# malak29/video-text-detection-system

Hardware: AMD Instinct MI355X
Metric: frames/sec (detect+recognize) @720p, 1/2/4/8 MI355X; box IoU vs CPU ref (higher is better)
Workload: dtype f16

## Files before the change

### include/vtd.h

```cpp
#ifndef VTD_H
#define VTD_H

#include <stddef.h>
#include <stdint.h>

#ifdef __cplusplus
extern "C" {
#endif

typedef struct vtd_detector vtd_detector;
typedef struct vtd_recognizer vtd_recognizer;
typedef struct vtd_postproc vtd_postproc;
typedef void* vtd_stream;

typedef struct vtd_detection {
    int32_t bbox[4];
    int32_t polygon[8];
    float confidence;
    float area;
    int32_t first_x, first_y;
} vtd_detection;

const char* vtd_version(void);
const char* vtd_strerror(int code);
int vtd_device_count(void);

int vtd_detector_create(const char* backbone, int max_batch, vtd_detector** out);
void vtd_detector_destroy(vtd_detector* d);
int vtd_detector_set_tensor(vtd_detector* d, const char* key, const float* host_data, int64_t numel);
int vtd_detector_set_option(vtd_detector* d, const char* name, int value);
int vtd_detector_finalize(vtd_detector* d, vtd_stream stream);
int vtd_detector_preprocess(vtd_detector* d, const uint8_t* frames_dev, int n, int height, int width, vtd_stream stream);
int vtd_detector_set_input_nchw(vtd_detector* d, const float* x_dev, int n, vtd_stream stream);
int vtd_detector_forward(vtd_detector* d, int n, float* prob_dev, float* thresh_dev, vtd_stream stream);
int vtd_detector_read_tap(vtd_detector* d, const char* name, int n, float* host_out, int64_t capacity, vtd_stream stream);
int64_t vtd_detector_macs_per_frame(const vtd_detector* d);
int vtd_detector_set_profiling(vtd_detector* d, int enable);
int vtd_detector_num_ops(const vtd_detector* d);
int vtd_detector_get_profile(vtd_detector* d, int op_index, char* name, int name_cap, double* total_ms, int64_t* calls,
                             double* total_macs, vtd_stream stream);

int vtd_detector_set_tuning(vtd_detector* d, const char* table_text);
int64_t vtd_detector_get_tuning(const vtd_detector* d, char* buf, int64_t capacity);
int vtd_detector_tuning_measured(const vtd_detector* d);

int vtd_postproc_create(int max_batch, int map_h, int map_w, int max_out, vtd_postproc** out);
void vtd_postproc_destroy(vtd_postproc* pp);
int vtd_postproc_run(vtd_postproc* pp, const float* prob_dev, int n, const int32_t* orig_w_host, const int32_t* orig_h_host,
                     float threshold, vtd_detection* out_dev, int32_t* counts_dev, vtd_stream stream);
int vtd_copy_to_pinned_host(const void* src_dev, void* dst_pinned_host, int64_t bytes, vtd_stream stream);

int64_t vtd_dbloss_workspace_bytes(void);
int vtd_dbloss_forward(const float* prob_dev, const float* thresh_dev, const float* prob_target_dev, const float* thresh_target_dev, int64_t numel,
                       float smooth, void* workspace_dev, float* out4_dev, double* sums5_dev, vtd_stream stream);
int vtd_dbloss_backward(const float* prob_dev, const float* thresh_dev, const float* prob_target_dev, const float* thresh_target_dev, int64_t numel,
                        float smooth, const double* sums5_dev, const float* grad_out4_dev, float* grad_prob_dev, float* grad_thresh_dev,
                        vtd_stream stream);
int vtd_binary_counts_accumulate(const float* pred_dev, const float* target_dev, int64_t numel, float threshold, int64_t* counts4_dev,
                                 vtd_stream stream);

#define VTD_ADAMW_SLICE 64
#define VTD_ADAMW_CHUNK 4096
typedef struct vtd_adamw_tensor {
    float* p;
    const float* g;
// ... 176 lines not shown
```

### video-text-detection-system_amd/csrc/detector_misc.hip

```cpp
#include "vtd_common.h"

namespace {

constexpr int PRE_TY = 16;
constexpr int PRE_OUT = 640;
constexpr int PRE_CHUNK = 4;
#ifndef VTD_PRE_NT
#define VTD_PRE_NT 640
#endif
constexpr int PRE_NT = VTD_PRE_NT;
constexpr int PRE_COLS = (PRE_OUT + PRE_NT - 1) / PRE_NT;

struct PreParams {
    const uint8_t* frames;
    half_t* out;
    const int* xb;
    const int* xk;
    const int* yb;
    const int* yk;
    int H, W, ksx, ksy;
    int max_rows;
    unsigned quads_magic;
};

// ... 188 lines not shown
        uint32_t acc[4][3];
#pragma unroll
        for (int q = 0; q < 4; ++q)
#pragma unroll
            for (int c = 0; c < 3; ++c) acc[q][c] = 1u << 21;
#pragma unroll
        for (int t = 0; t < KSY; ++t) {
            const uint32_t kv = (uint32_t)yt[2 + t];
            const int r = min(ymin + t, nrows - 1);
            const uint4 px = *(const uint4*)(rows + r * PRE_OUT + g * 4);
            const uint32_t pv[4] = {px.x, px.y, px.z, px.w};
#pragma unroll
            for (int q = 0; q < 4; ++q) {
                acc[q][0] = __umul24(pv[q] & 0xffu, kv) + acc[q][0];
                acc[q][1] = __umul24((pv[q] >> 8) & 0xffu, kv) + acc[q][1];
                acc[q][2] = __umul24(pv[q] >> 16, kv) + acc[q][2];
            }
        }
        half8 o01, o23;
#pragma unroll
        for (int q = 0; q < 4; ++q) {
            const half_t h0 = lut[clip8_22((int)acc[q][2])];
            const half_t h1 = lut[256 + clip8_22((int)acc[q][1])];
            const half_t h2 = lut[512 + clip8_22((int)acc[q][0])];
            if (q < 2) { o01[q * 4] = h0; o01[q * 4 + 1] = h1; o01[q * 4 + 2] = h2; o01[q * 4 + 3] = (half_t)0.f; }
            else { o23[(q - 2) * 4] = h0; o23[(q - 2) * 4 + 1] = h1; o23[(q - 2) * 4 + 2] = h2; o23[(q - 2) * 4 + 3] = (half_t)0.f; }
        }
        half_t* dst = p.out + (((int64_t)img * 646 + oy + 3) * 646 + g * 4 + 3) * 4;
        *(half4*)(dst) = half4{o01[0], o01[1], o01[2], o01[3]};
        *(half4*)(dst + 4) = half4{o01[4], o01[5], o01[6], o01[7]};
        *(half4*)(dst + 8) = half4{o23[0], o23[1], o23[2], o23[3]};
        *(half4*)(dst + 12) = half4{o23[4], o23[5], o23[6], o23[7]};
    }
}

__global__ void nchw_to_input_kernel(const float* __restrict__ x, half_t* __restrict__ out, int n) {
    const int64_t idx = (int64_t)blockIdx.x * blockDim.x + threadIdx.x;
    const int64_t total = (int64_t)n * 640 * 640;
    if (idx >= total) return;
    const int img = (int)(idx / (640 * 640));
    const int rem = (int)(idx - (int64_t)img * 640 * 640);
    const int y = rem / 640, xx = rem - y * 640;
    const float* base = x + (int64_t)img * 3 * 640 * 640 + rem;
    half4 o = {(half_t)base[0], (half_t)base[640 * 640], (half_t)base[2 * 640 * 640], (half_t)0.f};
    *(half4*)(out + (((int64_t)img * 646 + y + 3) * 646 + xx + 3) * 4) = o;
}

struct PoolParams {
    const half_t* in;
    half_t* out;
    int n, c, ho, wo;
    int in_hp, in_wp, in_y0, in_x0;
    int out_hp, out_wp, out_ring;
    int kh, kw, sh, sw;
};

__global__ void maxpool_kernel(const PoolParams p) {
    const int cg = p.c >> 3;
    const int64_t total = (int64_t)p.n * p.ho * p.wo * cg;
    for (int64_t idx = (int64_t)blockIdx.x * blockDim.x + threadIdx.x; idx < total; idx += (int64_t)gridDim.x * blockDim.x) {
        const int g = (int)(idx % cg);
        int64_t t = idx / cg;
        const int ox = (int)(t % p.wo);
        t /= p.wo;
        const int oy = (int)(t % p.ho);
        const int img = (int)(t / p.ho);
// ... 18 lines not shown
    PreParams p{frames, out, xb, xk, yb, yk, H, W, ksx, ksy, max_rows, 0u};
    if ((W & 3) == 0 && W <= 2048 && ksy == 5 && (ksx == 5 || ksx == 7)) {
        const int lds_fast = (max_rows * PRE_OUT + PRE_CHUNK * (W + ksx) + PRE_TY * (2 + ksy)) * 4 + 3 * 256 * 2;
        p.quads_magic = (unsigned)(((1ull << 32) + (W / 4) - 1) / (W / 4));
        if (lds_fast <= 160 * 1024) {
            static bool attr5 = false, attr7 = false;
            if (ksx == 5) {
                if (!attr5) {
                    VTD_HIP_CHECK(hipFuncSetAttribute((const void*)preprocess_fast_kernel<5, 5>, hipFuncAttributeMaxDynamicSharedMemorySize, 160 * 1024));
                    attr5 = true;
                }
                hipLaunchKernelGGL((preprocess_fast_kernel<5, 5>), dim3(PRE_OUT / PRE_TY, n), dim3(PRE_NT), lds_fast, stream, p);
            } else {
                if (!attr7) {
                    VTD_HIP_CHECK(hipFuncSetAttribute((const void*)preprocess_fast_kernel<7, 5>, hipFuncAttributeMaxDynamicSharedMemorySize, 160 * 1024));
                    attr7 = true;
                }
                hipLaunchKernelGGL((preprocess_fast_kernel<7, 5>), dim3(PRE_OUT / PRE_TY, n), dim3(PRE_NT), lds_fast, stream, p);
            }
            return -(int)hipGetLastError();
        }
    }
    const int lds = ((max_rows * PRE_OUT * 3 + 15) & ~15) + PRE_CHUNK * ((W * 3 + 15) & ~15);
    if (lds > 160 * 1024) return -1010;
    static bool attr_done = false;
    if (!attr_done) {
        VTD_HIP_CHECK(hipFuncSetAttribute((const void*)preprocess_kernel, hipFuncAttributeMaxDynamicSharedMemorySize, 160 * 1024));
        attr_done = true;
    }
    hipLaunchKernelGGL(preprocess_kernel, dim3(PRE_OUT / PRE_TY, n), dim3(256), lds, stream, p);
    return -(int)hipGetLastError();
}

int vtd_launch_nchw_to_input(const float* x, half_t* out, int n, hipStream_t stream) {
    const int64_t total = (int64_t)n * 640 * 640;
    hipLaunchKernelGGL(nchw_to_input_kernel, dim3((unsigned)((total + 255) / 256)), dim3(256), 0, stream, x, out, n);
    return -(int)hipGetLastError();
}

int vtd_launch_maxpool(const TensorDesc& in, const TensorDesc& out, int n, int kh, int kw, int sh, int sw, int pad_h, int pad_w,
                       hipStream_t stream) {
    if (in.c != out.c || (in.c & 7)) return -1020;
    if (in.ring < pad_h || in.ring < pad_w) return -1021;
    if ((out.h - 1) * sh - pad_h + kh > in.h + (in.hp - in.h - in.ring) || (out.w - 1) * sw - pad_w + kw > in.w + (in.wp - in.w - in.ring))
        return -1022;
    PoolParams p{in.ptr, out.ptr, n, in.c, out.h, out.w, in.hp, in.wp, in.ring - pad_h, in.ring - pad_w,
                 out.hp, out.wp, out.ring, kh, kw, sh, sw};
    const int64_t total = (int64_t)n * out.h * out.w * (in.c >> 3);
    const int blocks = (int)((total + 255) / 256 < 256 * 16 ? (total + 255) / 256 : 256 * 16);
    hipLaunchKernelGGL(maxpool_kernel, dim3(blocks), dim3(256), 0, stream, p);
    return -(int)hipGetLastError();
}
```

### video-text-detection-system_amd/csrc/recognizer.hip

```cpp
#include "../../include/vtd.h"
#include "vtd_common.h"

namespace {

struct CropParams {
    const uint8_t* frames;
    const int32_t* boxes;
    uint8_t* out;
    int H, W, ncrops;
};

__device__ __forceinline__ void linear_coef(int ssize, int dsize, int d, int& ofs, int& c0, int& c1) {
    const double scale = 1.0 / ((double)dsize / (double)ssize);
    float f = (float)(((double)d + 0.5) * scale - 0.5);
    int s = (int)floorf(f);
    f -= (float)s;
    if (s < 0) { f = 0.f; s = 0; }
    if (s >= ssize - 1) { f = 0.f; s = ssize - 1; }
    ofs = s;
    c0 = __float2int_rn((1.f - f) * 2048.f);
    c1 = __float2int_rn(f * 2048.f);
}

__global__ __launch_bounds__(256) void crop_resize_kernel(const CropParams p) {
    const int crop = blockIdx.x;
    const int32_t* b = p.boxes + crop * 5;
    const int x1 = b[1], y1 = b[2], sw = b[3] - b[1], sh = b[4] - b[2];
    uint8_t* dst = p.out + (int64_t)crop * 32 * 128 * 3;
    if (sw <= 0 || sh <= 0 || b[0] < 0 || x1 < 0 || y1 < 0 || b[3] > p.W || b[4] > p.H) {
        for (int i = threadIdx.x; i < 32 * 128 * 3; i += 256) dst[i] = 0;
        return;
    }
    const uint8_t* src = p.frames + ((int64_t)b[0] * p.H + y1) * p.W * 3 + (int64_t)x1 * 3;
    const int64_t stride = (int64_t)p.W * 3;
    const bool area = (sw == 256 && sh == 64);
    for (int i = threadIdx.x; i < 32 * 128; i += 256) {
        const int dy = i >> 7, dx = i & 127;
        if (area) {
            const uint8_t* r0 = src + (int64_t)(2 * dy) * stride + (2 * dx) * 3;
            const uint8_t* r1 = r0 + stride;
#pragma unroll
            for (int c = 0; c < 3; ++c) dst[i * 3 + c] = (uint8_t)((r0[c] + r0[3 + c] + r1[c] + r1[3 + c] + 2) >> 2);
            continue;
        }
        int sx0, a0, a1, sy0, b0, b1;
        linear_coef(sw, 128, dx, sx0, a0, a1);
        linear_coef(sh, 32, dy, sy0, b0, b1);
        const int sx1 = min(sx0 + 1, sw - 1), sy1 = min(sy0 + 1, sh - 1);
        const uint8_t* r0 = src + (int64_t)sy0 * stride;
        const uint8_t* r1 = src + (int64_t)sy1 * stride;
#pragma unroll
        for (int c = 0; c < 3; ++c) {
            const int h0 = r0[sx0 * 3 + c] * a0 + r0[sx1 * 3 + c] * a1;
            const int h1 = r1[sx0 * 3 + c] * a0 + r1[sx1 * 3 + c] * a1;
            int v = (((b0 * (h0 >> 4)) >> 16) + ((b1 * (h1 >> 4)) >> 16) + 2) >> 2;
            dst[i * 3 + c] = (uint8_t)(v < 0 ? 0 : (v > 255 ? 255 : v));
        }
    }
}

struct Conv1Params {
    const uint8_t* in_u8;
    const float* in_f32;
    const half_t* w;
    const float* bias;
    half_t* out;
    int n;
};

__global__ __launch_bounds__(256) void crnn_conv1_pool_kernel(const Conv1Params p) {
    __shared__ __attribute__((aligned(16))) half_t atile[256 * 32];
    __shared__ half_t tile[4][130][4];
    const int crop = blockIdx.y, py = blockIdx.x;
    for (int i = threadIdx.x; i < 4 * 130 * 3; i += 256) {
        const int c = i % 3, xx = (i / 3) % 130, r = i / (3 * 130);
        const int y = 2 * py - 1 + r, x = xx - 1;
        float v = 0.f;
        if (y >= 0 && y < 32 && x >= 0 && x < 128) {
            if (p.in_u8) v = (float)p.in_u8[(((int64_t)crop * 32 + y) * 128 + x) * 3 + c] / 255.0f;
            else v = p.in_f32[(((int64_t)crop * 3 + c) * 32 + y) * 128 + x];
        }
        tile[r][xx][c] = (half_t)v;
    }
    __syncthreads();
    {
        const int t = threadIdx.x, w = t >> 6, member = (t >> 4) & 3, win = t & 15;
        const int oy = member >> 1, ox = 2 * (w * 16 + win) + (member & 1);
        half_t vals[32];
#pragma unroll
// ... 244 lines not shown
```

### video-text-detection-system_amd/csrc/vtd_api.cpp

```cpp
#include <algorithm>
#include <cmath>
#include <cstdio>
#include <cstdlib>
#include <cstring>
#include <map>
#include <memory>
#include <string>
#include <vector>

#include "../../include/vtd.h"
#include "vtd_common.h"

int vtd_launch_conv(const ConvParams& p, int cfg, hipStream_t stream);
int vtd_conv_num_configs();
bool vtd_conv_config_valid(const ConvParams& p, int cfg);
int vtd_launch_preprocess(const uint8_t* frames, int n, int H, int W, half_t* out, const int* xb, const int* xk, int ksx,
                          const int* yb, const int* yk, int ksy, int max_rows, hipStream_t stream);
int vtd_launch_nchw_to_input(const float* x, half_t* out, int n, hipStream_t stream);
int vtd_launch_maxpool(const TensorDesc& in, const TensorDesc& out, int n, int kh, int kw, int sh, int sw, int pad_h, int pad_w,
                       hipStream_t stream);
void vtd_stem_pool_pack_weights(const float* w_folded, half_t* packed);
int vtd_launch_stem_pool(const TensorDesc& in, const TensorDesc& out, const half_t* w_packed, const float* bias, int n, hipStream_t stream);
extern "C" int vtd_head_entry_halo_steps(int py, int px, int nch1, int* out);
int vtd_launch_head_entry_halo(const ConvParams& c, const int* steps_dev, int nsteps, int big_tiles, hipStream_t stream);
#ifdef VTD_EXPERIMENTAL_CANDIDATES
extern "C" int vtd_head_entry_half_schedule(const int* steps, int nsteps, int* out);
int vtd_launch_head_entry_half(const ConvParams& c, const int* sched_dev, int nsteps, hipStream_t stream);
int vtd_head_entry_pair_tables(int py, int px, int c2ch, int* half_steps, int* plan);
int vtd_launch_head_entry_pair(const ConvParams& c, const int* half_steps_dev, const int* plan_dev, int nh, hipStream_t stream);
#endif
bool vtd_conv_halo_supported(const ConvParams& c, int* bn_out, int* tw_out);
bool vtd_conv_halo_c64_supported(const ConvParams& c, int tw);
int vtd_launch_conv_halo(const ConvParams& c, int bn, int tw, hipStream_t stream);
bool vtd_pointwise128_supported(const ConvParams& c);
int vtd_launch_pointwise128(const ConvParams& c, hipStream_t stream);
void vtd_head_tail_pack_w1(const half_t* w1_gemm, half_t* packed);
void vtd_head_tail_pack_w2(const float* w2, half_t* packed);
int vtd_launch_head_tail(const TensorDesc& in, const half_t* w1, const float* bias1, const half_t* w2, float b2, float* out, int n,
                         hipStream_t stream);

int vtd_launch_crop_resize(const uint8_t* frames, int H, int W, const int32_t* boxes, int ncrops, uint8_t* out, hipStream_t s);
int vtd_launch_crnn_conv1(const uint8_t* in_u8, const float* in_f32, const half_t* w, const float* bias, half_t* out, int n, hipStream_t s);
int vtd_launch_lstm(const half_t* xs, const half_t* whh, half_t* hout, int D, int T, hipStream_t s);
int vtd_launch_ctc_greedy(const float* logits, int n, int T, int V, int ld, const int32_t* id2char, int blank, int apply_softmax,
                          int32_t* out, hipStream_t s);
int vtd_launch_compact_rows(const float* in, float* out, int64_t rows, int V, int ld, hipStream_t s);
int vtd_dbloss_ws_bytes();
int vtd_launch_dbloss(const float* prob, const float* thresh, const float* prob_t, const float* thresh_t, int64_t n, float smooth, double* workspace,
                      float* out4, double* sums5, hipStream_t stream);
int vtd_launch_dbloss_backward(const float* prob, const float* thresh, const float* prob_t, const float* thresh_t, int64_t n, float smooth,
// ... 379 lines not shown
    ResampleAxis a;
    const double scale = (double)in_size / out_size;
    const double fscale = scale < 1.0 ? 1.0 : scale;
    const double support = fscale;
    a.ksize = (int)std::ceil(support) * 2 + 1;
    a.bounds.assign(2 * (size_t)out_size, 0);
    a.kk.assign((size_t)out_size * a.ksize, 0);
    std::vector<double> pre(a.ksize);
    for (int xx = 0; xx < out_size; ++xx) {
        const double center = (xx + 0.5) * scale, ss = 1.0 / fscale;
        int xmin = (int)(center - support + 0.5);
        if (xmin < 0) xmin = 0;
        int xmax = (int)(center + support + 0.5);
        if (xmax > in_size) xmax = in_size;
        xmax -= xmin;
        double ww = 0.0;
        for (int x = 0; x < xmax; ++x) {
            double t = (x + xmin - center + 0.5) * ss;
            if (t < 0) t = -t;
            const double wv = t < 1.0 ? 1.0 - t : 0.0;
            pre[x] = wv;
            ww += wv;
        }
        for (int x = 0; x < xmax; ++x) {
            const double v = ww != 0.0 ? pre[x] / ww : pre[x];
            a.kk[(size_t)xx * a.ksize + x] = v < 0 ? (int)(-0.5 + v * (1 << 22)) : (int)(0.5 + v * (1 << 22));
        }
        a.bounds[2 * xx] = xmin;
        a.bounds[2 * xx + 1] = xmax;
    }
    return a;
}

struct PreTables {
    int *xb = nullptr, *xk = nullptr, *yb = nullptr, *yk = nullptr;
    int ksx = 0, ksy = 0, max_rows = 0;
};

}

using namespace vtd;

namespace vtd {
struct ModelBase {
    StateDict sd;
    DeviceArena arena;
    std::map<std::string, int> tuning;
    bool tuning_measured = false;
    int alloc_tensor(TensorDesc& t) {
        void* p = nullptr;
        int rc = arena.alloc(&p, (size_t)tensor_elems(t) * sizeof(half_t), true);
        t.ptr = (half_t*)p;
        return rc;
    }
    const std::vector<float>* get(const std::string& k, size_t numel) const {
        auto it = sd.find(k);
        if (it == sd.end() || it->second.size() != numel) return nullptr;
        return &it->second;
    }
};

static std::string conv_signature(const ConvOp& c) {
    char buf[192];
    int len = std::snprintf(buf, sizeof buf, "conv|in%dx%dx%d|out%dx%d|co%d|K%d|s%d|f%x|r%d|c%d", c.in.h, c.in.w, c.in.c, c.ho, c.wo, c.cout, c.K,
                            c.stride, (unsigned)c.flags, c.has_res ? 1 + c.res_shift : 0, c.plist ? 1 : 0);
    if (c.dual) len += std::snprintf(buf + len, sizeof buf - len, "|x%dm%ds%d", c.in2.c, c.in2_mul, c.in2_shr);
    if (c.pool_pw) std::snprintf(buf + len, sizeof buf - len, "|p2x%d", c.pool_pw);
    return buf;
}
// ... 57 lines not shown
        m->tuning[line.substr(0, ke)] = (int)v;
    }
    return 0;
}

static int64_t get_tuning_text(const ModelBase* m, char* buf, int64_t cap) {
    if (!m) return ERR_ARG;
    std::string out;
    for (const auto& kv : m->tuning) out += kv.first + " " + std::to_string(kv.second) + "\n";
    if (buf && cap > 0) {
        const size_t ncopy = std::min((size_t)cap - 1, out.size());
        std::memcpy(buf, out.data(), ncopy);
        buf[ncopy] = 0;
    }
    return (int64_t)out.size() + 1;
}

static int batch_bucket(int n, int cap) {
    int b = 1;
    while (b < n) b <<= 1;
    return std::min(b, cap);
}

}

struct vtd_detector : vtd::ModelBase {
    std::string backbone;
    int max_batch = 0;
    bool finalized = false;
    std::vector<Op> ops;
    TensorDesc input;
    std::map<std::string, TensorDesc> taps;
    std::map<std::pair<int, int>, PreTables> pre;
    int64_t macs = 0;
    float* final_out[2] = {nullptr, nullptr};
    std::map<int, std::vector<int>> tuned;
    bool head_tail_kernel = true;
    bool fuse_stem_pool = true;
    bool fuse_fpn_head = true;
    bool fuse_downsample = true;
    size_t pool_ops = 0;
    size_t trunk_ops = 0;
    size_t p2_ops = 0;
    bool profiling = false;
    int prof_only = -1;
    std::vector<hipEvent_t> ev_pool;
    size_t ev_used = 0;
    std::vector<std::pair<int, std::pair<hipEvent_t, hipEvent_t>>> ev_spans;
    std::vector<double> prof_ms;
    std::vector<int64_t> prof_calls;
    std::vector<double> prof_macs;
    hipEvent_t take_event() {
        if (ev_used == ev_pool.size()) {
            hipEvent_t e;
            if (hipEventCreate(&e) != hipSuccess) return nullptr;
            ev_pool.push_back(e);
        }
        return ev_pool[ev_used++];
    }
    ~vtd_detector() {
        for (hipEvent_t e : ev_pool) (void)hipEventDestroy(e);
    }
};


struct vtd_recognizer : vtd::ModelBase {
// ... 687 lines not shown
    if ((rc = upload(d->arena, b.data(), b.size() * sizeof(float), (void**)&op.bias))) return rc;
    op.in = in; op.out = in; op.K = K; op.cout = N; op.cout_pad = cout_pad; op.stride = 1;
    op.in_y0 = in.ring; op.in_x0 = in.ring; op.flags = out_flag; op.ho = in.h; op.wo = in.w;
    op.out_f32 = out_f32; op.ldc = ldc;
    op.macs_per_image = (int64_t)in.h * in.w * N * K;
    return 0;
}

static bool known_detector_key(const std::string& k) {
    return k.rfind("backbone.", 0) == 0 || k.rfind("fpn.", 0) == 0 || k.rfind("head.", 0) == 0;
}

static int get_pre_tables(vtd_detector* d, int H, int W, PreTables& out) {
    auto key = std::make_pair(H, W);
    auto it = d->pre.find(key);
    if (it != d->pre.end()) {
        out = it->second;
        return 0;
    }
    ResampleAxis ax = pillow_axis(W, 640), ay = pillow_axis(H, 640);
    PreTables t;
    t.ksx = ax.ksize; t.ksy = ay.ksize;
    int max_rows = 0;
    for (int oy0 = 0; oy0 < 640; oy0 += 16) {
        const int last = std::min(oy0 + 16, 640) - 1;
        max_rows = std::max(max_rows, ay.bounds[2 * last] + ay.bounds[2 * last + 1] - ay.bounds[2 * oy0]);
    }
    t.max_rows = max_rows;
    int rc;
    if ((rc = upload(d->arena, ax.bounds.data(), ax.bounds.size() * sizeof(int), (void**)&t.xb))) return rc;
    if ((rc = upload(d->arena, ax.kk.data(), ax.kk.size() * sizeof(int), (void**)&t.xk))) return rc;
    if ((rc = upload(d->arena, ay.bounds.data(), ay.bounds.size() * sizeof(int), (void**)&t.yb))) return rc;
    if ((rc = upload(d->arena, ay.kk.data(), ay.kk.size() * sizeof(int), (void**)&t.yk))) return rc;
    d->pre[key] = t;
    out = t;
    return 0;
}

}

extern "C" {

const char* vtd_version(void) {
#ifdef VTD_EXPERIMENTAL_CANDIDATES
    return "vtd_hip 0.3 (gfx950) +experimental";
#else
    return "vtd_hip 0.3 (gfx950)";
#endif
}

const char* vtd_strerror(int code) {
    static thread_local char buf[128];
    switch (code) {
        case 0: return "ok";
        case ERR_ARG: return "invalid argument";
        case ERR_UNKNOWN_KEY: return "unknown state-dict key";
        case ERR_SHAPE: return "tensor has the wrong number of elements";
        case ERR_MISSING_KEY: return "state dict incomplete (missing or mis-sized key)";
        case ERR_NOT_FINALIZED: return "handle not finalized";
        case ERR_BATCH: return "batch exceeds the handle's max_batch";
        case ERR_GEOMETRY: return "layer geometry check failed";
        case ERR_CAPACITY: return "output capacity too small";
        case -2801: return "feature export needs a detector finalized with fuse_fpn_head=0 (the fused head entry never forms P2)";
        case -2802: return "DB head training: invalid argument or shape";
        case -2803: return "DB head training: misaligned buffer";
        case -2901: return "trunk export needs a detector finalized with fuse_fpn_head=0 (the fused graph pads C2 for the composed head entry)";
// ... 256 lines not shown
    if (b != "resnet18" && b != "resnet50") return ERR_ARG;
    auto* d = new vtd_detector();
    d->backbone = b;
    d->max_batch = max_batch;
    *out = d;
    return 0;
}

void vtd_detector_destroy(vtd_detector* d) { delete d; }

int vtd_detector_set_tensor(vtd_detector* d, const char* key, const float* host_data, int64_t numel) {
    if (!d || !key || !host_data || numel < 0) return ERR_ARG;
    const std::string k = key;
    if (!known_detector_key(k)) return ERR_UNKNOWN_KEY;
    if (k.size() > 19 && k.compare(k.size() - 19, 19, "num_batches_tracked") == 0) return 0;
    d->sd[k].assign(host_data, host_data + numel);
    return 0;
}

int vtd_detector_set_option(vtd_detector* d, const char* name, int value) {
    if (!d || !name || d->finalized) return ERR_ARG;
    if (std::string(name) == "fuse_fpn_head") { d->fuse_fpn_head = value != 0; return 0; }
    if (std::string(name) == "fuse_stem_pool") { d->fuse_stem_pool = value != 0; return 0; }
    if (std::string(name) == "head_tail_kernel") { d->head_tail_kernel = value != 0; return 0; }
    if (std::string(name) == "fuse_downsample") { d->fuse_downsample = value != 0; return 0; }
    return ERR_UNKNOWN_KEY;
}

int vtd_detector_finalize(vtd_detector* d, vtd_stream stream) {
    if (!d) return ERR_ARG;
    if (d->finalized) return ERR_ARG;
    int rc = build_detector_graph(d);
    if (rc) return rc;
    hipError_t e = hipStreamSynchronize((hipStream_t)stream);
    if (e != hipSuccess) return -(int)e;
    d->sd.clear();
    d->finalized = true;
    return 0;
}

int vtd_detector_preprocess(vtd_detector* d, const uint8_t* frames_dev, int n, int height, int width, vtd_stream stream) {
    if (!d || !frames_dev || height <= 0 || width <= 0) return ERR_ARG;
    if (!d->finalized) return ERR_NOT_FINALIZED;
    if (n <= 0 || n > d->max_batch) return ERR_BATCH;
    PreTables t;
    int rc = get_pre_tables(d, height, width, t);
    if (rc) return rc;
    return vtd_launch_preprocess(frames_dev, n, height, width, d->input.ptr, t.xb, t.xk, t.ksx, t.yb, t.yk, t.ksy, t.max_rows,
                                 (hipStream_t)stream);
}

int vtd_detector_set_input_nchw(vtd_detector* d, const float* x_dev, int n, vtd_stream stream) {
    if (!d || !x_dev) return ERR_ARG;
    if (!d->finalized) return ERR_NOT_FINALIZED;
    if (n <= 0 || n > d->max_batch) return ERR_BATCH;
    return vtd_launch_nchw_to_input(x_dev, d->input.ptr, n, (hipStream_t)stream);
}

static int run_detector_ops(vtd_detector* d, int n, float* prob_dev, float* thresh_dev, hipStream_t s, size_t op_end) {
    float* outs[2] = {prob_dev, thresh_dev};
    const int bucket = batch_bucket(n, d->max_batch);
    auto tit = d->tuned.find(bucket);
    if (tit == d->tuned.end()) {
        std::vector<int> cfgs(d->ops.size(), -1);
        for (size_t oi = 0; oi < d->ops.size(); ++oi)
            if (d->ops[oi].kind == Op::CONV) {
                int rc = choose_config(d, d->ops[oi].conv, bucket, s, &cfgs[oi]);
                if (rc) return rc;
            }
        tit = d->tuned.emplace(bucket, std::move(cfgs)).first;
    }
    const std::vector<int>& cfgs = tit->second;
    for (size_t oi = 0; oi < op_end; ++oi) {
        const Op& o = d->ops[oi];
        int rc = 0;
        if (o.final_slot == 1 && !thresh_dev) continue;
        if (o.kind == Op::BORDER && (oi == 0 || (cfgs[oi - 1] != kHeadEntryHaloCfg && cfgs[oi - 1] != kHeadEntryHalo256Cfg && cfgs[oi - 1] != kHeadEntryPairCfg && cfgs[oi - 1] != kHeadEntryHalfCfg)))
            continue;
        hipEvent_t e0 = nullptr, e1 = nullptr;
        const bool prof = d->profiling && (d->prof_only < 0 || d->prof_only == (int)oi);
        if (prof) {
            e0 = d->take_event();
// ... 430 lines not shown
```

### video-text-detection-system_amd/vtd_amd/_native.py

```python
import ctypes as C
import os

_HERE = os.path.dirname(os.path.abspath(__file__))
_VARIANT = os.environ.get("VTD_LIB_VARIANT", "")
LIB_PATH = os.path.join(_HERE, "_lib", f"libvtd_hip_{_VARIANT}.so" if _VARIANT else "libvtd_hip.so")

_lib = None


class NativeError(RuntimeError):
    pass


class TrocrConfig(C.Structure):
    _fields_ = [("image_size", C.c_int32), ("patch_size", C.c_int32), ("enc_hidden", C.c_int32), ("enc_layers", C.c_int32),
                ("enc_heads", C.c_int32), ("enc_ffn", C.c_int32), ("enc_qkv_bias", C.c_int32), ("enc_ln_eps", C.c_float),
                ("dec_hidden", C.c_int32), ("dec_layers", C.c_int32), ("dec_heads", C.c_int32), ("dec_ffn", C.c_int32),
                ("vocab_size", C.c_int32), ("max_positions", C.c_int32), ("dec_ln_eps", C.c_float),
                ("decoder_start_token_id", C.c_int32), ("eos_token_id", C.c_int32), ("pad_token_id", C.c_int32), ("max_length", C.c_int32)]


class Detection(C.Structure):
    _fields_ = [("bbox", C.c_int32 * 4), ("polygon", C.c_int32 * 8), ("confidence", C.c_float), ("area", C.c_float),
                ("first_x", C.c_int32), ("first_y", C.c_int32)]
# ... 19 lines not shown
class BasicBlockParams(C.Structure):
    _fields_ = [(k, C.c_void_p) for k in BLOCK_FIELDS]


class StemParams(C.Structure):
    _fields_ = [(k, C.c_void_p) for k in ("w", "gamma", "beta", "mean", "var")]


FpnTaps = C.c_void_p * 4

ADAMW_SLICE = 64
ADAMW_CHUNK = 4096


class AdamwTensor(C.Structure):
    _fields_ = [("p", C.c_void_p), ("g", C.c_void_p), ("m", C.c_void_p), ("v", C.c_void_p), ("n", C.c_int64), ("step_size", C.c_float),
                ("bc2_sqrt", C.c_float)]


class AdamwHyper(C.Structure):
    _fields_ = [(k, C.c_float) for k in ("decay", "one_minus_beta1", "beta2", "one_minus_beta2", "eps")]


SIGNATURES = {
    "vtd_version": (C.c_char_p, []),
    "vtd_strerror": (C.c_char_p, [C.c_int]),
    "vtd_device_count": (C.c_int, []),
    "vtd_detector_create": (C.c_int, [C.c_char_p, C.c_int, C.POINTER(C.c_void_p)]),
    "vtd_detector_destroy": (None, [C.c_void_p]),
    "vtd_detector_set_tensor": (C.c_int, [C.c_void_p, C.c_char_p, C.c_void_p, C.c_int64]),
    "vtd_detector_set_option": (C.c_int, [C.c_void_p, C.c_char_p, C.c_int]),
    "vtd_detector_finalize": (C.c_int, [C.c_void_p, C.c_void_p]),
    "vtd_detector_preprocess": (C.c_int, [C.c_void_p, C.c_void_p, C.c_int, C.c_int, C.c_int, C.c_void_p]),
    "vtd_detector_set_input_nchw": (C.c_int, [C.c_void_p, C.c_void_p, C.c_int, C.c_void_p]),
    "vtd_detector_forward": (C.c_int, [C.c_void_p, C.c_int, C.c_void_p, C.c_void_p, C.c_void_p]),
    "vtd_detector_read_tap": (C.c_int, [C.c_void_p, C.c_char_p, C.c_int, C.c_void_p, C.c_int64, C.c_void_p]),
    "vtd_detector_macs_per_frame": (C.c_int64, [C.c_void_p]),
    "vtd_detector_set_profiling": (C.c_int, [C.c_void_p, C.c_int]),
    "vtd_detector_num_ops": (C.c_int, [C.c_void_p]),
    "vtd_detector_get_profile": (C.c_int, [C.c_void_p, C.c_int, C.c_char_p, C.c_int, C.POINTER(C.c_double), C.POINTER(C.c_int64),
                                           C.POINTER(C.c_double), C.c_void_p]),
    "vtd_detector_set_tuning": (C.c_int, [C.c_void_p, C.c_char_p]),
    "vtd_detector_get_tuning": (C.c_int64, [C.c_void_p, C.c_char_p, C.c_int64]),
    "vtd_detector_tuning_measured": (C.c_int, [C.c_void_p]),
    "vtd_postproc_create": (C.c_int, [C.c_int, C.c_int, C.c_int, C.c_int, C.POINTER(C.c_void_p)]),
    "vtd_postproc_destroy": (None, [C.c_void_p]),
    "vtd_copy_to_pinned_host": (C.c_int, [C.c_void_p, C.c_void_p, C.c_int64, C.c_void_p]),
    "vtd_postproc_run": (C.c_int, [C.c_void_p, C.c_void_p, C.c_int, C.c_void_p, C.c_void_p, C.c_float, C.c_void_p, C.c_void_p,
                                   C.c_void_p]),
    "vtd_recognizer_create": (C.c_int, [C.c_int, C.c_int, C.POINTER(C.c_void_p)]),
    "vtd_recognizer_set_option": (C.c_int, [C.c_void_p, C.c_char_p, C.c_int]),
    "vtd_recognizer_destroy": (None, [C.c_void_p]),
    "vtd_recognizer_set_tensor": (C.c_int, [C.c_void_p, C.c_char_p, C.c_void_p, C.c_int64]),
    "vtd_recognizer_finalize": (C.c_int, [C.c_void_p, C.c_void_p]),
    "vtd_recognizer_crop_resize": (C.c_int, [C.c_void_p, C.c_void_p, C.c_int, C.c_int, C.c_int, C.c_void_p, C.c_int, C.c_void_p]),
    "vtd_recognizer_set_input_nchw": (C.c_int, [C.c_void_p, C.c_void_p, C.c_int, C.c_void_p]),
    "vtd_recognizer_forward": (C.c_int, [C.c_void_p, C.c_int, C.c_void_p, C.c_void_p]),
    "vtd_recognizer_read_tap": (C.c_int, [C.c_void_p, C.c_char_p, C.c_int, C.c_void_p, C.c_int64, C.c_void_p]),
    "vtd_recognizer_macs_per_crop": (C.c_int64, [C.c_void_p]),
    "vtd_recognizer_set_tuning": (C.c_int, [C.c_void_p, C.c_char_p]),
    "vtd_recognizer_get_tuning": (C.c_int64, [C.c_void_p, C.c_char_p, C.c_int64]),
    "vtd_recognizer_tuning_measured": (C.c_int, [C.c_void_p]),
    "vtd_trocr_create": (C.c_int, [C.c_void_p, C.c_int, C.POINTER(C.c_void_p)]),
    "vtd_trocr_destroy": (None, [C.c_void_p]),
    "vtd_trocr_set_tensor": (C.c_int, [C.c_void_p, C.c_char_p, C.c_void_p, C.c_int64]),
    "vtd_trocr_finalize": (C.c_int, [C.c_void_p, C.c_void_p]),
# ... 121 lines not shown
```

Baseline: 12570.

## Add banded tiled preprocess kernel with trimmed resample taps and LDS ring

Measured after the change: 12670 (median of 6 runs). Within noise of the previous version (+0.8%).

```diff
diff --git a/include/vtd.h b/include/vtd.h
--- a/include/vtd.h
+++ b/include/vtd.h
@@ -31,6 +31,7 @@
 int vtd_detector_set_option(vtd_detector* d, const char* name, int value);
 int vtd_detector_finalize(vtd_detector* d, vtd_stream stream);
 int vtd_detector_preprocess(vtd_detector* d, const uint8_t* frames_dev, int n, int height, int width, vtd_stream stream);
+int vtd_preprocess_plan(int height, int width, int* info, int kcap, int* xmin, int* xcoef, int* ymin, int* ycoef);
 int vtd_detector_set_input_nchw(vtd_detector* d, const float* x_dev, int n, vtd_stream stream);
 int vtd_detector_forward(vtd_detector* d, int n, float* prob_dev, float* thresh_dev, vtd_stream stream);
 int vtd_detector_read_tap(vtd_detector* d, const char* name, int n, float* host_out, int64_t capacity, vtd_stream stream);
diff --git a/video-text-detection-system_amd/csrc/detector_misc.hip b/video-text-detection-system_amd/csrc/detector_misc.hip
--- a/video-text-detection-system_amd/csrc/detector_misc.hip
+++ b/video-text-detection-system_amd/csrc/detector_misc.hip
@@ -244,6 +244,174 @@
         *(half4*)(dst + 8) = half4{o23[0], o23[1], o23[2], o23[3]};
         *(half4*)(dst + 12) = half4{o23[4], o23[5], o23[6], o23[7]};
     }
+}
+
+constexpr int PB_BANDS = 8, PB_STRIPS = 4;
+constexpr int PB_ROWS = PRE_OUT / PB_BANDS, PB_COLS = PRE_OUT / PB_STRIPS;
+constexpr int PB_NT = 2 * PB_COLS, PB_CHUNK = 4, PB_RING = 16;
+constexpr int PB_PLAN_Q0 = 0, PB_PLAN_NQ = PB_STRIPS, PB_PLAN_Y0 = 2 * PB_STRIPS, PB_PLAN_NROWS = 2 * PB_STRIPS + PB_BANDS;
+
+struct PreBandParams {
+    const uint8_t* frames;
+    half_t* out;
+    const int* xmin;
+    const int* xk;
+    const int* yb;
+    const int* yk;
+    const int* plan;
+    int H, W;
+    int pitch;
+};
+
+__device__ __forceinline__ void pb_lds_barrier() {
+    asm volatile("s_waitcnt lgkmcnt(0)" ::: "memory");
+    __builtin_amdgcn_s_barrier();
+    asm volatile("" ::: "memory");
+}
+
+template <int KSX, int KSY>
+__global__ __launch_bounds__(PB_NT) void preprocess_bands_kernel(const PreBandParams p) {
+    extern __shared__ __attribute__((aligned(16))) uint8_t lds[];
+    constexpr int YT = 2 + KSY;
+    uint32_t* const ring = (uint32_t*)lds;
+    uint32_t* const raw = ring + PB_RING * PB_COLS;
+    const int pitch = p.pitch;
+    int* const ytab = (int*)(raw + 2 * PB_CHUNK * pitch);
+    half_t* const lut = (half_t*)(ytab + (PB_ROWS + 4) * YT);
+    const int strip = blockIdx.x, band = blockIdx.y, img = blockIdx.z;
+    const int tid = threadIdx.x;
+    const int q0 = p.plan[PB_PLAN_Q0 + strip], nq = p.plan[PB_PLAN_NQ + strip];
+    const int y_first = p.plan[PB_PLAN_Y0 + band], nrows = p.plan[PB_PLAN_NROWS + band];
+    const int oy0 = band * PB_ROWS, ox0 = strip * PB_COLS;
+    const int row_bytes = p.W * 3;
+    const uint8_t* src = p.frames + ((int64_t)img * p.H + y_first) * row_bytes + (int64_t)q0 * 12;
+    const int nchunks = (nrows + PB_CHUNK - 1) / PB_CHUNK;
+
+    const int hc = tid % PB_COLS, hr = tid / PB_COLS;
+    const int xrel = p.xmin[ox0 + hc] - 4 * q0;
+    uint32_t kx[KSX];
+#pragma unroll
+    for (int t = 0; t < KSX; ++t) kx[t] = (uint32_t)p.xk[(ox0 + hc) * KSX + t];
+    for (int i = tid; i < (PB_ROWS + 4) * YT; i += PB_NT) {
+        const int ty = i / YT, e = i - ty * YT;
+        const int oy = oy0 + ty;
+        ytab[i] = ty >= PB_ROWS ? (e == 1 ? 0x7fffffff : 0) : (e < 2 ? p.yb[2 * oy + e] - y_first : p.yk[oy * KSY + (e - 2)]);
+    }
+    for (int i = tid; i < PB_RING * PB_COLS + 2 * PB_CHUNK * pitch; i += PB_NT) ring[i] = 0u;
+    {
+        const float mean[3] = {0.485f, 0.456f, 0.406f};
+        const float stdv[3] = {0.229f, 0.224f, 0.225f};
+        if (tid < 256) {
+#pragma unroll
+            for (int c = 0; c < 3; ++c) lut[c * 256 + tid] = (half_t)(((float)tid / 255.0f - mean[c]) / stdv[c]);
+        }
+    }
+
+    const int fq = min(hc, nq - 1);
+    uint32_t stg0[2][3], stg1[2][3];
+    auto fetch = [&](int c, uint32_t (&stg)[2][3]) {
+#pragma unroll
+        for (int j = 0; j < 2; ++j) {
+            const int r = min(c * PB_CHUNK + hr + 2 * j, nrows - 1);
+            const uint32_t* g = (const uint32_t*)(src + (int64_t)r * row_bytes) + fq * 3;
+            stg[j][0] = g[0]; stg[j][1] = g[1]; stg[j][2] = g[2];
+        }
+    };
+    auto stage = [&](int c, uint32_t (&stg)[2][3]) {
+        uint32_t* const dst = raw + (c & 1) * PB_CHUNK * pitch;
+#pragma unroll
+        for (int j = 0; j < 2; ++j) {
+            const int rr = hr + 2 * j;
+            if (hc < nq && c * PB_CHUNK + rr < nrows) {
+                const uint32_t d0 = stg[j][0], d1 = stg[j][1], d2 = stg[j][2];
+                uint4 px;
+                px.x = d0 & 0xffffffu;
+                px.y = ((d0 >> 24) | (d1 << 8)) & 0xffffffu;
+                px.z = ((d1 >> 16) | (d2 << 16)) & 0xffffffu;
+                px.w = d2 >> 8;
+                *(uint4*)(dst + rr * pitch + hc * 4) = px;
+            }
+        }
+    };
+    auto horiz = [&](int c) {
+        const uint32_t* const srcb = raw + (c & 1) * PB_CHUNK * pitch + xrel;
+#pragma unroll
+        for (int j = 0; j < 2; ++j) {
+            const int rr = hr + 2 * j, r = c * PB_CHUNK + rr;
+            if (r < nrows) {
+                const uint32_t* row = srcb + rr * pitch;
+                uint32_t s0 = 1u << 21, s1 = 1u << 21, s2 = 1u << 21;
+#pragma unroll
+                for (int t = 0; t < KSX; ++t) {
+                    const uint32_t px = row[t];
+                    s0 = __umul24(px & 0xffu, kx[t]) + s0;
+                    s1 = __umul24((px >> 8) & 0xffu, kx[t]) + s1;
+                    s2 = __umul24(px >> 16, kx[t]) + s2;
+                }
+                ring[(r & (PB_RING - 1)) * PB_COLS + hc] =
+                    (uint32_t)clip8_22((int)s0) | ((uint32_t)clip8_22((int)s1) << 8) | ((uint32_t)clip8_22((int)s2) << 16);
+            }
+        }
+    };
+    const int vp = tid % (PB_COLS / 2), vs = tid / (PB_COLS / 2);
+    int o_next = 0;
+    auto vert = [&](int done) -> int {
+        {
+            int cnt = 0;
+#pragma unroll
+            for (int s = 0; s < 4; ++s) cnt += ytab[(o_next + s) * YT + 1] <= done ? 1 : 0;
+            if (vs < cnt) {
+                const int ty = o_next + vs;
+                const int* yt = ytab + ty * YT;
+                const int ymin = yt[0];
+                uint32_t acc[2][3];
+#pragma unroll
+                for (int q = 0; q < 2; ++q)
+#pragma unroll
+                    for (int c = 0; c < 3; ++c) acc[q][c] = 1u << 21;
+#pragma unroll
+                for (int t = 0; t < KSY; ++t) {
+                    const uint32_t kv = (uint32_t)yt[2 + t];
+                    const uint2 px = *(const uint2*)(ring + ((ymin + t) & (PB_RING - 1)) * PB_COLS + vp * 2);
+                    const uint32_t pv[2] = {px.x, px.y};
+#pragma unroll
+                    for (int q = 0; q < 2; ++q) {
+                        acc[q][0] = __umul24(pv[q] & 0xffu, kv) + acc[q][0];
+                        acc[q][1] = __umul24((pv[q] >> 8) & 0xffu, kv) + acc[q][1];
+                        acc[q][2] = __umul24(pv[q] >> 16, kv) + acc[q][2];
+                    }
+                }
+                half_t* dst = p.out + (((int64_t)img * 646 + oy0 + ty + 3) * 646 + ox0 + vp * 2 + 3) * 4;
+#pragma unroll
+                for (int q = 0; q < 2; ++q)
+                    *(half4*)(dst + q * 4) = half4{lut[clip8_22((int)acc[q][2])], lut[256 + clip8_22((int)acc[q][1])],
+                                                   lut[512 + clip8_22((int)acc[q][0])], (half_t)0.f};
+            }
+            o_next += cnt;
+            return cnt;
+        }
+    };
+
+    fetch(0, stg0);
+    fetch(1, stg1);
+    pb_lds_barrier();
+    stage(0, stg0);
+    fetch(2, stg0);
+    pb_lds_barrier();
+    auto step = [&](int c, uint32_t (&stg)[2][3]) {
+        stage(c + 1, stg);
+        const int done = min(nrows, c * PB_CHUNK);
+        vert(done);
+        vert(done);
+        fetch(c + 3, stg);
+        horiz(c);
+        pb_lds_barrier();
+    };
+    for (int c = 0; c < nchunks; c += 2) {
+        step(c, stg1);
+        step(c + 1, stg0);
+    }
+    while (vert(nrows) == 4) {}
 }
 
 __global__ void nchw_to_input_kernel(const float* __restrict__ x, half_t* __restrict__ out, int n) {
@@ -328,6 +496,25 @@
     return -(int)hipGetLastError();
 }
 
+int vtd_launch_preprocess_bands(const uint8_t* frames, int n, int H, int W, half_t* out, const int* xmin, const int* xk, int ksx,
+                                const int* yb, const int* yk, int ksy, const int* plan, int pitch, hipStream_t stream) {
+    const PreBandParams p{frames, out, xmin, xk, yb, yk, plan, H, W, pitch};
+    const int lds = (PB_RING * PB_COLS + 2 * PB_CHUNK * pitch + (PB_ROWS + 4) * (2 + ksy)) * 4 + 3 * 256 * 2;
+    if ((W & 3) || (pitch & 3) || lds > 48 * 1024 || n <= 0 || n > 65535) return -1011;
+    const dim3 grid(PB_STRIPS, PB_BANDS, n), block(PB_NT);
+#define VTD_PB_CASE(KX, KY) \
+    if (ksx == KX && ksy == KY) { \
+        hipLaunchKernelGGL((preprocess_bands_kernel<KX, KY>), grid, block, lds, stream, p); \
+        return -(int)hipGetLastError(); \
+    }
+    VTD_PB_CASE(3, 3) VTD_PB_CASE(3, 4) VTD_PB_CASE(3, 5)
+    VTD_PB_CASE(4, 3) VTD_PB_CASE(4, 4) VTD_PB_CASE(4, 5)
+    VTD_PB_CASE(5, 3) VTD_PB_CASE(5, 4) VTD_PB_CASE(5, 5)
+    VTD_PB_CASE(7, 3) VTD_PB_CASE(7, 4) VTD_PB_CASE(7, 5)
+#undef VTD_PB_CASE
+    return -1012;
+}
+
 int vtd_launch_nchw_to_input(const float* x, half_t* out, int n, hipStream_t stream) {
     const int64_t total = (int64_t)n * 640 * 640;
     hipLaunchKernelGGL(nchw_to_input_kernel, dim3((unsigned)((total + 255) / 256)), dim3(256), 0, stream, x, out, n);
diff --git a/video-text-detection-system_amd/csrc/recognizer.hip b/video-text-detection-system_amd/csrc/recognizer.hip
--- a/video-text-detection-system_amd/csrc/recognizer.hip
+++ b/video-text-detection-system_amd/csrc/recognizer.hip
@@ -34,27 +34,56 @@
     const uint8_t* src = p.frames + ((int64_t)b[0] * p.H + y1) * p.W * 3 + (int64_t)x1 * 3;
     const int64_t stride = (int64_t)p.W * 3;
     const bool area = (sw == 256 && sh == 64);
-    for (int i = threadIdx.x; i < 32 * 128; i += 256) {
-        const int dy = i >> 7, dx = i & 127;
-        if (area) {
+    __shared__ int4 coef[128 + 32];
+    if (!area) {
+        if (threadIdx.x < 128 + 32) {
+            const bool col = threadIdx.x < 128;
+            const int ssize = col ? sw : sh;
+            int ofs, c0, c1;
+            linear_coef(ssize, col ? 128 : 32, col ? (int)threadIdx.x : (int)threadIdx.x - 128, ofs, c0, c1);
+            coef[threadIdx.x] = make_int4(ofs, c0, c1, min(ofs + 1, ssize - 1));
+        }
+        __syncthreads();
+    }
+    if (area) {
+        for (int i = threadIdx.x; i < 32 * 128; i += 256) {
+            const int dy = i >> 7, dx = i & 127;
             const uint8_t* r0 = src + (int64_t)(2 * dy) * stride + (2 * dx) * 3;
             const uint8_t* r1 = r0 + stride;
 #pragma unroll
             for (int c = 0; c < 3; ++c) dst[i * 3 + c] = (uint8_t)((r0[c] + r0[3 + c] + r1[c] + r1[3 + c] + 2) >> 2);
-            continue;
-        }
-        int sx0, a0, a1, sy0, b0, b1;
-        linear_coef(sw, 128, dx, sx0, a0, a1);
-        linear_coef(sh, 32, dy, sy0, b0, b1);
-        const int sx1 = min(sx0 + 1, sw - 1), sy1 = min(sy0 + 1, sh - 1);
-        const uint8_t* r0 = src + (int64_t)sy0 * stride;
-        const uint8_t* r1 = src + (int64_t)sy1 * stride;
-#pragma unroll
-        for (int c = 0; c < 3; ++c) {
-            const int h0 = r0[sx0 * 3 + c] * a0 + r0[sx1 * 3 + c] * a1;
-            const int h1 = r1[sx0 * 3 + c] * a0 + r1[sx1 * 3 + c] * a1;
-            int v = (((b0 * (h0 >> 4)) >> 16) + ((b1 * (h1 >> 4)) >> 16) + 2) >> 2;
-            dst[i * 3 + c] = (uint8_t)(v < 0 ? 0 : (v > 255 ? 255 : v));
+        }
+        return;
+    }
+    constexpr int CROP_U = 8;
+    const int dx = threadIdx.x & 127, dyb = threadIdx.x >> 7;
+    const int4 cx = coef[dx];
+    const int sx0 = cx.x * 3, a0 = cx.y, a1 = cx.z, sx1 = cx.w * 3;
+    for (int k0 = 0; k0 < 16; k0 += CROP_U) {
+        uint8_t px[CROP_U][4][3];
+        int b0[CROP_U], b1[CROP_U];
+#pragma unroll
+        for (int u = 0; u < CROP_U; ++u) {
+            const int4 cy = coef[128 + dyb + 2 * (k0 + u)];
+            b0[u] = cy.y; b1[u] = cy.z;
+            const uint8_t* r0 = src + (int64_t)cy.x * stride;
+            const uint8_t* r1 = src + (int64_t)cy.w * stride;
+#pragma unroll
+            for (int c = 0; c < 3; ++c) {
+                px[u][0][c] = r0[sx0 + c]; px[u][1][c] = r0[sx1 + c];
+                px[u][2][c] = r1[sx0 + c]; px[u][3][c] = r1[sx1 + c];
+            }
+        }
+#pragma unroll
+        for (int u = 0; u < CROP_U; ++u) {
+            const int i = (dyb + 2 * (k0 + u)) * 128 + dx;
+#pragma unroll
+            for (int c = 0; c < 3; ++c) {
+                const int h0 = px[u][0][c] * a0 + px[u][1][c] * a1;
+                const int h1 = px[u][2][c] * a0 + px[u][3][c] * a1;
+                int v = (((b0[u] * (h0 >> 4)) >> 16) + ((b1[u] * (h1 >> 4)) >> 16) + 2) >> 2;
+                dst[i * 3 + c] = (uint8_t)(v < 0 ? 0 : (v > 255 ? 255 : v));
+            }
         }
     }
 }
diff --git a/video-text-detection-system_amd/csrc/vtd_api.cpp b/video-text-detection-system_amd/csrc/vtd_api.cpp
--- a/video-text-detection-system_amd/csrc/vtd_api.cpp
+++ b/video-text-detection-system_amd/csrc/vtd_api.cpp
@@ -16,6 +16,8 @@
 bool vtd_conv_config_valid(const ConvParams& p, int cfg);
 int vtd_launch_preprocess(const uint8_t* frames, int n, int H, int W, half_t* out, const int* xb, const int* xk, int ksx,
                           const int* yb, const int* yk, int ksy, int max_rows, hipStream_t stream);
+int vtd_launch_preprocess_bands(const uint8_t* frames, int n, int H, int W, half_t* out, const int* xmin, const int* xk, int ksx,
+                                const int* yb, const int* yk, int ksy, const int* plan, int pitch, hipStream_t stream);
 int vtd_launch_nchw_to_input(const float* x, half_t* out, int n, hipStream_t stream);
 int vtd_launch_maxpool(const TensorDesc& in, const TensorDesc& out, int n, int kh, int kw, int sh, int sw, int pad_h, int pad_w,
                        hipStream_t stream);
@@ -461,9 +463,107 @@
     return a;
 }
 
+constexpr int kPreBands = 8, kPreStrips = 4, kPreChunk = 4, kPreRing = 16, kPreLdsMax = 48 * 1024;
+struct PrePlan {
+    bool fast = false;
+    int tx = 0, ty = 0, ksx = 0, ksy = 0, pitch = 0, lds_bytes = 0;
+    int64_t rows_resampled = 0;
+    std::vector<int> xmin, xcnt, xk, ymin, ycnt, yk;
+    std::vector<int> dxk, dyb, dyk, plan;
+};
+
+static void trim_axis(const ResampleAxis& a, int out_size, std::vector<int>& first, std::vector<int>& count, std::vector<int>& kk, int& widest) {
+    first.assign(out_size, 0);
+    count.assign(out_size, 1);
+    std::vector<int> lo(out_size, 0);
+    widest = 1;
+    for (int o = 0; o < out_size; ++o) {
+        const int* k = a.kk.data() + (size_t)o * a.ksize;
+        const int cnt = a.bounds[2 * o + 1];
+        int l = 0, h = cnt - 1;
+        while (l < h && k[l] == 0) ++l;
+        while (h > l && k[h] == 0) --h;
+        lo[o] = l;
+        first[o] = a.bounds[2 * o] + l;
+        count[o] = std::max(1, h - l + 1);
+        widest = std::max(widest, count[o]);
+    }
+    kk.assign((size_t)out_size * widest, 0);
+    for (int o = 0; o < out_size; ++o)
+        for (int t = 0; t < count[o]; ++t) kk[(size_t)o * widest + t] = a.kk[(size_t)o * a.ksize + lo[o] + t];
+}
+
+static int pre_instance(int widest, std::initializer_list<int> built) {
+    for (int b : built)
+        if (widest <= b) return b;
+    return 0;
+}
+
+static PrePlan plan_preprocess(int H, int W) {
+    const int N = 640, cols = N / kPreStrips, rows = N / kPreBands;
+    PrePlan p;
+    const ResampleAxis ax = pillow_axis(W, N), ay = pillow_axis(H, N);
+    trim_axis(ax, N, p.xmin, p.xcnt, p.xk, p.tx);
+    trim_axis(ay, N, p.ymin, p.ycnt, p.yk, p.ty);
+    p.ksx = pre_instance(p.tx, {3, 4, 5, 7});
+    p.ksy = pre_instance(p.ty, {3, 4, 5});
+    bool ok = (W & 3) == 0 && W <= 2048 && p.ksx && p.ksy;
+    const int sx = std::max(p.ksx, p.tx), sy = std::max(p.ksy, p.ty);
+    p.dxk.assign((size_t)N * sx, 0);
+    p.dyk.assign((size_t)N * sy, 0);
+    for (int o = 0; o < N; ++o) {
+        for (int t = 0; t < p.xcnt[o]; ++t) p.dxk[(size_t)o * sx + t] = p.xk[(size_t)o * p.tx + t];
+        for (int t = 0; t < p.ycnt[o]; ++t) p.dyk[(size_t)o * sy + t] = p.yk[(size_t)o * p.ty + t];
+    }
+    p.plan.assign(2 * kPreStrips + 2 * kPreBands, 0);
+    int pitch = 4;
+    for (int s = 0; s < kPreStrips; ++s) {
+        int lo = W, hi = 0;
+        for (int o = s * cols; o < (s + 1) * cols; ++o) {
+            lo = std::min(lo, p.xmin[o]);
+            hi = std::max(hi, p.xmin[o] + p.xcnt[o]);
+        }
+        const int q0 = lo / 4, nq = (hi + 3) / 4 - q0;
+        p.plan[s] = q0;
+        p.plan[kPreStrips + s] = nq;
+        if (nq > cols || 4 * (q0 + nq) > W) ok = false;
+        pitch = std::max(pitch, 4 * nq);
+        for (int o = s * cols; o < (s + 1) * cols; ++o) pitch = std::max(pitch, p.xmin[o] - 4 * q0 + sx);
+    }
+    p.pitch = (pitch + 3) & ~3;
+    p.dyb.assign(2 * (size_t)N, 0);
+    for (int b = 0; b < kPreBands; ++b) {
+        int y0 = H, y1 = 0;
+        for (int o = b * rows; o < (b + 1) * rows; ++o) {
+            y0 = std::min(y0, p.ymin[o]);
+            y1 = std::max(y1, p.ymin[o] + p.ycnt[o]);
+            p.dyb[2 * o] = p.ymin[o];
+            p.dyb[2 * o + 1] = y1;
+        }
+        p.plan[2 * kPreStrips + b] = y0;
+        p.plan[2 * kPreStrips + kPreBands + b] = y1 - y0;
+        p.rows_resampled += y1 - y0;
+        const int nrows = y1 - y0, nchunks = (nrows + kPreChunk - 1) / kPreChunk;
+        int o = b * rows;
+        for (int c = 0; c < ((nchunks + 1) & ~1); ++c) {
+            const int done = std::min(nrows, kPreChunk * c), newest = std::min(nrows, kPreChunk * (c + 1)) - 1;
+            for (int k = 0; k < 8 && o < (b + 1) * rows && p.dyb[2 * o + 1] - y0 <= done; ++k, ++o)
+                if (p.ymin[o] - y0 + kPreRing <= newest) ok = false;
+        }
+        for (; o < (b + 1) * rows; ++o)
+            if (p.ymin[o] - y0 + kPreRing <= nrows - 1) ok = false;
+    }
+    p.lds_bytes = (kPreRing * cols + 2 * kPreChunk * p.pitch + (rows + 4) * (2 + p.ksy)) * 4 + 3 * 256 * 2;
+    p.fast = ok && p.lds_bytes <= kPreLdsMax;
+    return p;
+}
+
 struct PreTables {
     int *xb = nullptr, *xk = nullptr, *yb = nullptr, *yk = nullptr;
     int ksx = 0, ksy = 0, max_rows = 0;
+    bool bands = false;
+    int *bxmin = nullptr, *bxk = nullptr, *byb = nullptr, *byk = nullptr, *bplan = nullptr;
+    int bksx = 0, bksy = 0, bpitch = 0;
 };
 
 }
@@ -587,6 +687,7 @@
     TensorDesc input;
     std::map<std::string, TensorDesc> taps;
     std::map<std::pair<int, int>, PreTables> pre;
+    bool pre_tiled = false;
     int64_t macs = 0;
     float* final_out[2] = {nullptr, nullptr};
     std::map<int, std::vector<int>> tuned;
@@ -1340,6 +1441,18 @@
     if ((rc = upload(d->arena, ax.kk.data(), ax.kk.size() * sizeof(int), (void**)&t.xk))) return rc;
     if ((rc = upload(d->arena, ay.bounds.data(), ay.bounds.size() * sizeof(int), (void**)&t.yb))) return rc;
     if ((rc = upload(d->arena, ay.kk.data(), ay.kk.size() * sizeof(int), (void**)&t.yk))) return rc;
+    if (!d->pre_tiled) {
+        const PrePlan pl = plan_preprocess(H, W);
+        if (pl.fast) {
+            t.bands = true;
+            t.bksx = pl.ksx; t.bksy = pl.ksy; t.bpitch = pl.pitch;
+            if ((rc = upload(d->arena, pl.xmin.data(), pl.xmin.size() * sizeof(int), (void**)&t.bxmin))) return rc;
+            if ((rc = upload(d->arena, pl.dxk.data(), pl.dxk.size() * sizeof(int), (void**)&t.bxk))) return rc;
+            if ((rc = upload(d->arena, pl.dyb.data(), pl.dyb.size() * sizeof(int), (void**)&t.byb))) return rc;
+            if ((rc = upload(d->arena, pl.dyk.data(), pl.dyk.size() * sizeof(int), (void**)&t.byk))) return rc;
+            if ((rc = upload(d->arena, pl.plan.data(), pl.plan.size() * sizeof(int), (void**)&t.bplan))) return rc;
+        }
+    }
     d->pre[key] = t;
     out = t;
     return 0;
@@ -1662,6 +1775,7 @@
     if (d->finalized) return ERR_ARG;
     int rc = build_detector_graph(d);
     if (rc) return rc;
+    if (const char* e = std::getenv("VTD_PRE_TILED"); e && e[0] == '1') d->pre_tiled = true;
     hipError_t e = hipStreamSynchronize((hipStream_t)stream);
     if (e != hipSuccess) return -(int)e;
     d->sd.clear();
@@ -1676,8 +1790,28 @@
     PreTables t;
     int rc = get_pre_tables(d, height, width, t);
     if (rc) return rc;
+    if (t.bands)
+        return vtd_launch_preprocess_bands(frames_dev, n, height, width, d->input.ptr, t.bxmin, t.bxk, t.bksx, t.byb, t.byk, t.bksy, t.bplan,
+                                           t.bpitch, (hipStream_t)stream);
     return vtd_launch_preprocess(frames_dev, n, height, width, d->input.ptr, t.xb, t.xk, t.ksx, t.yb, t.yk, t.ksy, t.max_rows,
                                  (hipStream_t)stream);
+}
+
+int vtd_preprocess_plan(int height, int width, int* info, int kcap, int* xmin, int* xcoef, int* ymin, int* ycoef) {
+    if (height <= 0 || width <= 0 || !info || kcap <= 0 || !xmin || !xcoef || !ymin || !ycoef) return ERR_ARG;
+    const PrePlan p = plan_preprocess(height, width);
+    if (p.tx > kcap || p.ty > kcap) return ERR_CAPACITY;
+    const int v[8] = {p.fast ? 1 : 0, p.tx, p.ty, p.ksx, p.ksy, p.lds_bytes, (int)p.rows_resampled, kPreBands * kPreStrips};
+    std::copy(v, v + 8, info);
+    std::fill(xcoef, xcoef + (size_t)640 * kcap, 0);
+    std::fill(ycoef, ycoef + (size_t)640 * kcap, 0);
+    for (int o = 0; o < 640; ++o) {
+        xmin[o] = p.xmin[o];
+        ymin[o] = p.ymin[o];
+        for (int t = 0; t < p.xcnt[o]; ++t) xcoef[(size_t)o * kcap + t] = p.xk[(size_t)o * p.tx + t];
+        for (int t = 0; t < p.ycnt[o]; ++t) ycoef[(size_t)o * kcap + t] = p.yk[(size_t)o * p.ty + t];
+    }
+    return 0;
 }
 
 int vtd_detector_set_input_nchw(vtd_detector* d, const float* x_dev, int n, vtd_stream stream) {
diff --git a/video-text-detection-system_amd/vtd_amd/_native.py b/video-text-detection-system_amd/vtd_amd/_native.py
--- a/video-text-detection-system_amd/vtd_amd/_native.py
+++ b/video-text-detection-system_amd/vtd_amd/_native.py
@@ -75,6 +75,7 @@
     "vtd_detector_set_option": (C.c_int, [C.c_void_p, C.c_char_p, C.c_int]),
     "vtd_detector_finalize": (C.c_int, [C.c_void_p, C.c_void_p]),
     "vtd_detector_preprocess": (C.c_int, [C.c_void_p, C.c_void_p, C.c_int, C.c_int, C.c_int, C.c_void_p]),
+    "vtd_preprocess_plan": (C.c_int, [C.c_int, C.c_int, C.c_void_p, C.c_int, C.c_void_p, C.c_void_p, C.c_void_p, C.c_void_p]),
     "vtd_detector_set_input_nchw": (C.c_int, [C.c_void_p, C.c_void_p, C.c_int, C.c_void_p]),
     "vtd_detector_forward": (C.c_int, [C.c_void_p, C.c_int, C.c_void_p, C.c_void_p, C.c_void_p]),
     "vtd_detector_read_tap": (C.c_int, [C.c_void_p, C.c_char_p, C.c_int, C.c_void_p, C.c_int64, C.c_void_p]),
```
